# PTsolvers/JustRelax.jl

Measured on AMD Instinct MI355X. Metric: PT-iterations/s (3D Stokes SolVi3D, 512^3 fp64 block per GPU, block-iterations summed over GPUs), higher is better.
Workload: dtype f64; 1 GPU; SolVi3D 512^3 per GPU (configs[3]): eta inclusion 1e-3, G=1, K=Inf, dt=Inf, free-slip, pure shear; kernel_form=viscous_limit_no_body_forces, halo=none, arrays=library constructor, field_placement=1 (pool-dealt chunks, mapped once), operand_cache=0

## Files before the change

### justrelax.jl_amd/csrc/jrx_kernels.hpp

```cpp
#pragma once
#include "jrx_internal.hpp"

namespace {

__global__ __launch_bounds__(256) void k_scale3(double *__restrict__ U0, const double *__restrict__ V0, i64 n0,
                                                double *__restrict__ U1, const double *__restrict__ V1, i64 n1,
                                                double *__restrict__ U2, const double *__restrict__ V2, i64 n2, double dt)
{
    const i64 stride = (i64)gridDim.x * blockDim.x;
    for (i64 t = (i64)blockIdx.x * blockDim.x + threadIdx.x; t < n0 || t < n1 || t < n2; t += stride) {
        if (t < n0) U0[t] = V0[t] * dt;
        if (t < n1) U1[t] = V1[t] * dt;
        if (U2 && t < n2) U2[t] = V2[t] * dt;
    }
}

struct BcArr {
    double *p;
    int n[3];
};

__global__ __launch_bounds__(256) void k_bc3d(BcArr A0, BcArr A1, BcArr A2, int type, int dim, int lo_on, int hi_on)
{
    const BcArr arrs[3] = {A0, A1, A2};
// ... 19 lines not shown
                if (hi_on) p[base + (e - 1) * s[dim]] = 0.0;
            } else {
                if (lo_on) p[base] = -p[base + s[dim]];
                if (hi_on) p[base + (e - 1) * s[dim]] = -p[base + (e - 2) * s[dim]];
            }
        } else {
            if (normal) {
                if (lo_on) p[base] = p[base + (e - 1) * s[dim]];
            } else {
                if (lo_on) p[base] = p[base + (e - 2) * s[dim]];
                if (hi_on) p[base + (e - 1) * s[dim]] = p[base + s[dim]];
            }
        }
    }
}

struct CBcArr {
    const double *p;
    int n[3];
};
__global__ __launch_bounds__(256) void k_copy_shell3(BcArr D0, BcArr D1, BcArr D2, CBcArr S0, CBcArr S1, CBcArr S2)
{
    const BcArr D = blockIdx.z == 0 ? D0 : (blockIdx.z == 1 ? D1 : D2);
    const CBcArr S = blockIdx.z == 0 ? S0 : (blockIdx.z == 1 ? S1 : S2);
    const int dim = blockIdx.y >> 1, side = blockIdx.y & 1;
    const int d1 = dim == 0 ? 1 : 0, d2 = dim == 2 ? 1 : 2;
    const i64 u = (i64)blockIdx.x * blockDim.x + threadIdx.x;
    if (u >= (i64)D.n[d1] * D.n[d2]) return;
    const int a = (int)(u % D.n[d1]), b = (int)(u / D.n[d1]);
    const i64 s[3] = {1, D.n[0], (i64)D.n[0] * D.n[1]};
    const i64 idx = a * s[d1] + b * s[d2] + (side ? (i64)(D.n[dim] - 1) * s[dim] : 0);
    D.p[idx] = S.p[idx];
}

__global__ __launch_bounds__(256) void k_bc3d_faces(BcArr A0, BcArr A1, BcArr A2, int tlo0, int thi0, int tlo1, int thi1, int tlo2, int thi2)
{
    const BcArr arrs[3] = {A0, A1, A2};
    const int dim = blockIdx.z;
    const int tlo = dim == 0 ? tlo0 : (dim == 1 ? tlo1 : tlo2), thi = dim == 0 ? thi0 : (dim == 1 ? thi1 : thi2);
    if (!tlo && !thi) return;
    const int d1 = dim == 0 ? 1 : 0, d2 = dim == 2 ? 1 : 2;
    const int ta = blockIdx.x * blockDim.x + threadIdx.x;
    const int tb = blockIdx.y;
#pragma unroll
    for (int c = 0; c < 3; c++) {
        const BcArr &A = arrs[c];
        if (ta >= A.n[d1] || tb >= A.n[d2]) continue;
        const bool normal = (c == dim);
        const i64 s[3] = {1, A.n[0], (i64)A.n[0] * A.n[1]};
        const i64 base = ta * s[d1] + tb * s[d2];
        const int e = A.n[dim];
        double *p = A.p;
        if (normal) {
            if (tlo == 2) p[base] = 0.0;
            if (thi == 2) p[base + (e - 1) * s[dim]] = 0.0;
        } else {
            if (tlo == 1) p[base] = p[base + s[dim]];
            else if (tlo == 2) p[base] = -p[base + s[dim]];
            if (thi == 1) p[base + (e - 1) * s[dim]] = p[base + (e - 2) * s[dim]];
            else if (thi == 2) p[base + (e - 1) * s[dim]] = -p[base + (e - 2) * s[dim]];
        }
    }
}

__global__ __launch_bounds__(256) void k_maxloc(double *__restrict__ B, const double *__restrict__ A, int nx, int ny, int nz)
{
    const int t = blockIdx.x * blockDim.x + threadIdx.x;
    const int j = t / nx, i = t - j * nx, k = blockIdx.y;
    if (j >= ny) return;
    double x = -INFINITY;
    for (int kk = k - 1; kk <= k + 1; kk++) {
        const int kc = clampi(kk, 0, nz - 1);
        for (int jj = j - 1; jj <= j + 1; jj++) {
            const int jc = clampi(jj, 0, ny - 1);
            for (int ii = i - 1; ii <= i + 1; ii++) {
                const int ic = clampi(ii, 0, nx - 1);
                const double v = A[ic + (i64)nx * jc + (i64)nx * ny * kc];
                if (v > x) x = v;
            }
        }
    }
    B[i + (i64)nx * j + (i64)nx * ny * k] = x;
}

struct RedArr {
    const double *p;
    int n[3];
    int inner;
};

__global__ __launch_bounds__(256) void k_sumsq_partial(RedArr A0, RedArr A1, RedArr A2, RedArr A3, double *__restrict__ partials)
{
    const RedArr arrs[4] = {A0, A1, A2, A3};
    __shared__ double sm[4][4];
    const int lane = threadIdx.x & 63, wave = threadIdx.x >> 6;
    const i64 stride = (i64)gridDim.x * blockDim.x;
#pragma unroll
    for (int c = 0; c < 4; c++) {
        const RedArr &A = arrs[c];
        double s = 0.0;
        if (A.p) {
            const i64 n = (i64)A.n[0] * A.n[1] * A.n[2];
            for (i64 t = (i64)blockIdx.x * blockDim.x + threadIdx.x; t < n; t += stride) {
                bool take = true;
                if (A.inner) {
                    const int i = (int)(t % A.n[0]);
                    const i64 q = t / A.n[0];
                    const int j = (int)(q % A.n[1]);
                    const int k = (int)(q / A.n[1]);
                    take = i > 0 && i < A.n[0] - 1 && j > 0 && j < A.n[1] - 1 && (A.n[2] == 1 || (k > 0 && k < A.n[2] - 1));
                }
                if (take) {
                    const double v = A.p[t];
                    s += v * v;
                }
            }
        }
        s = wave_sum(s);
        if (lane == 0) sm[c][wave] = s;
    }
    __syncthreads();
    if (threadIdx.x < 4) {
        const int c = threadIdx.x;
        partials[(i64)blockIdx.x * 4 + c] = (sm[c][0] + sm[c][1]) + (sm[c][2] + sm[c][3]);
    }
}

__global__ __launch_bounds__(256) void k_sumsq_final(const double *__restrict__ partials, int nblocks, double *__restrict__ out)
{
    __shared__ double sm[4][4];
    const int lane = threadIdx.x & 63, wave = threadIdx.x >> 6;
#pragma unroll
    for (int c = 0; c < 4; c++) {
        double s = 0.0;
        for (int b = threadIdx.x; b < nblocks; b += blockDim.x) s += partials[(i64)b * 4 + c];
        s = wave_sum(s);
        if (lane == 0) sm[c][wave] = s;
    }
    __syncthreads();
    if (threadIdx.x < 4) {
        const int c = threadIdx.x;
        out[c] = (sm[c][0] + sm[c][1]) + (sm[c][2] + sm[c][3]);
    }
}

__global__ __launch_bounds__(256) void k_maxabs_partial(const double *__restrict__ A0, i64 n0, const double *__restrict__ A1, i64 n1,
                                                        const double *__restrict__ A2, i64 n2, double *__restrict__ partials)
{
    __shared__ double sm[3][4];
    const double *A[3] = {A0, A1, A2};
    const i64 n[3] = {n0, n1, n2};
    const int lane = threadIdx.x & 63, wave = threadIdx.x >> 6;
    const i64 stride = (i64)gridDim.x * blockDim.x;
#pragma unroll
    for (int c = 0; c < 3; c++) {
        double m = 0.0;
        if (A[c])
            for (i64 t = (i64)blockIdx.x * blockDim.x + threadIdx.x; t < n[c]; t += stride) {
                const double v = fabs(A[c][t]);
                m = (v > m || v != v) ? v : m;
            }
#pragma unroll
        for (int off = 32; off > 0; off >>= 1) {
            const double o = __shfl_down(m, off, 64);
            m = (o > m || o != o) ? o : m;
        }
// ... 69 lines not shown
```

### justrelax.jl_amd/csrc/stokes3d.hip

```cpp
#include <vector>
#include <cstdlib>
#include "jrx_internal.hpp"
#include "jrx_kernels.hpp"
#include "stokes3d_kernels.hpp"
#include "jrx_tuning.h"

namespace {

SweepArgs make_args(const jrx_stokes3d_fields *f, const double *etatau, const jrx_stokes3d_params *p)
{
    SweepArgs a;
    a.f = *f;
    a.o = Out10{f->P, f->txx, f->tyy, f->tzz, f->tyz, f->txz, f->txy, f->Vx, f->Vy, f->Vz};
    a.etatau = etatau;
    a._dx = p->_dx; a._dy = p->_dy; a._dz = p->_dz;
    a.dt = p->dt; a.r = p->r; a.theta_dtau = p->theta_dtau; a.eta_dtau = p->eta_dtau;
    a.L = make_lay((int)p->nx, (int)p->ny, (int)p->nz);
    a.i0 = a.j0 = a.k0 = 0;
    a.i1 = a.j1 = a.k1 = 0;
    return a;
}

jrx_status check_params(jrx_handle *h, const jrx_stokes3d_fields *f, const jrx_stokes3d_params *p)
{
    if (!h) return JRX_ERR_ARG;
    if (!f || !p) return jrx_fail(h, JRX_ERR_ARG, "null fields/params");
    JRX_TRY(jrx_check_device(h));
    if (p->nx < 3 || p->ny < 3 || p->nz < 3) return jrx_fail(h, JRX_ERR_ARG, "3D Stokes needs at least 3 cells per dimension");
    const double cells = (double)(p->nx + 2) * (double)(p->ny + 2) * (double)(p->nz + 2);
    if (cells >= 2147483647.0) return jrx_fail(h, JRX_ERR_UNSUPPORTED, "local block too large for 32-bit plane indices");
    const void *req[] = {f->P, f->P0, f->Q, f->Vx, f->Vy, f->Vz, f->txx, f->tyy, f->tzz, f->tyz, f->txz, f->txy,
                         f->toxx, f->toyy, f->tozz, f->toyz, f->toxz, f->toxy, f->eta, f->K, f->G, f->fx, f->fy, f->fz};
    for (const void *q : req)
        if (!q) return jrx_fail(h, JRX_ERR_ARG, "a required field pointer is NULL");
    return JRX_OK;
}

jrx_status check_diag(jrx_handle *h, const jrx_stokes3d_fields *f)
{
    const void *req[] = {f->divV, f->exx, f->eyy, f->ezz, f->eyz, f->exz, f->exy, f->RP, f->Rx, f->Ry, f->Rz, f->Ux, f->Uy, f->Uz};
    for (const void *q : req)
        if (!q) return jrx_fail(h, JRX_ERR_ARG, "a diagnostic field pointer (∇V, ε, R, U) is NULL");
    return JRX_OK;
}

jrx_status launch_stress_v1(jrx_handle *h, hipStream_t s, SweepArgs a, bool diag, int i0, int i1, int j0, int j1, int k0, int k1)
{
    if (i1 <= i0 || j1 <= j0 || k1 <= k0) return JRX_OK;
    a.i0 = i0; a.i1 = i1; a.j0 = j0; a.j1 = j1; a.k0 = k0; a.k1 = k1;
    const i64 plane = (i64)(i1 - i0) * (j1 - j0);
    dim3 grid((unsigned)((plane + 255) / 256), (unsigned)(k1 - k0));
    if (diag) hipLaunchKernelGGL(k_stress3d<true>, grid, dim3(256), 0, s, a);
    else hipLaunchKernelGGL(k_stress3d<false>, grid, dim3(256), 0, s, a);
    JRX_LAUNCH_CHECK(h);
    return JRX_OK;
}

jrx_status launch_velocity_v1(jrx_handle *h, hipStream_t s, SweepArgs a, bool diag, int i0, int i1, int j0, int j1, int k0, int k1)
{
    if (i1 <= i0 || j1 <= j0 || k1 <= k0) return JRX_OK;
    a.i0 = i0; a.i1 = i1; a.j0 = j0; a.j1 = j1; a.k0 = k0; a.k1 = k1;
    const i64 plane = (i64)(i1 - i0) * (j1 - j0);
    dim3 grid((unsigned)((plane + 255) / 256), (unsigned)(k1 - k0));
    if (diag) hipLaunchKernelGGL(k_velocity3d<true>, grid, dim3(256), 0, s, a);
    else hipLaunchKernelGGL(k_velocity3d<false>, grid, dim3(256), 0, s, a);
    JRX_LAUNCH_CHECK(h);
    return JRX_OK;
}

bool fits_u32(const Lay3 &L)
{
    const double m = (double)(L.nx + 2) * (double)(L.ny + 2) * (double)(L.nz + 2) * 8.0;
    return m < 4294967296.0;
}

template <class F>
__device__ __forceinline__ void scan_pairs(const double *__restrict__ p, i64 n, F f)
{
    if (n <= 0) return;
    const i64 stride = (i64)gridDim.x * blockDim.x, t0 = (i64)blockIdx.x * blockDim.x + threadIdx.x;
    const i64 head = (reinterpret_cast<uintptr_t>(p) & 15) ? 1 : 0;
    const double2 *__restrict__ q = reinterpret_cast<const double2 *>(p + head);
    const i64 m = n - head;
    for (i64 t = t0; t < (m >> 1); t += stride) { const double2 v = q[t]; f(v.x); f(v.y); }
    if (t0 == 0) { if (head) f(p[0]); if (m & 1) f(p[n - 1]); }
}
__global__ __launch_bounds__(256) void k_visc_operands_ok(const double *__restrict__ c0, const double *__restrict__ c1, const double *__restrict__ c2, const double *__restrict__ c3,
                                                          const double *__restrict__ c4, const double *__restrict__ eta, i64 nc, const double *__restrict__ K, const double *__restrict__ G,
                                                          const double *__restrict__ yz, i64 nyz, const double *__restrict__ xz, i64 nxz, const double *__restrict__ xy, i64 nxy, int *bad,
                                                          const unsigned long long *__restrict__ fx, const unsigned long long *__restrict__ fy, const unsigned long long *__restrict__ fz)
{
    bool b = false;
    unsigned long long bxy = 0, bz = 0;
    auto fin = [&](double v) { b |= !isfinite(v); };
    auto mod = [&](double v) { b |= (v != v) || v == 0.0; };
    scan_pairs(c0, nc, fin); scan_pairs(c1, nc, fin); scan_pairs(c2, nc, fin); scan_pairs(c3, nc, fin); scan_pairs(c4, nc, fin); scan_pairs(eta, nc, fin);
    scan_pairs(K, nc, mod); scan_pairs(G, nc, mod);
    scan_pairs(yz, nyz, fin); scan_pairs(xz, nxz, fin); scan_pairs(xy, nxy, fin);
    if (fx) {
        scan_pairs(reinterpret_cast<const double *>(fx), nc, [&](double v) { bxy |= (unsigned long long)__double_as_longlong(v); });
        scan_pairs(reinterpret_cast<const double *>(fy), nc, [&](double v) { bxy |= (unsigned long long)__double_as_longlong(v); });
        scan_pairs(reinterpret_cast<const double *>(fz), nc, [&](double v) { bz |= (unsigned long long)__double_as_longlong(v); });
    }
    if (__any(b) && (threadIdx.x & 63) == 0) atomicOr(bad, 1);
    if (fx) {
        const int m = (__any(bxy != 0) ? 2 : 0) | (__any(bz != 0) ? 4 : 0);
        if (m && (threadIdx.x & 63) == 0) atomicOr(bad, m);
    }
}

__global__ __launch_bounds__(256) void k_forces_zero(const unsigned long long *__restrict__ fx, const unsigned long long *__restrict__ fy, const unsigned long long *__restrict__ fz, i64 nc, int *bad)
{
    const i64 stride = (i64)gridDim.x * blockDim.x;
    unsigned long long bxy = 0, bz = 0;
    for (i64 t = (i64)blockIdx.x * blockDim.x + threadIdx.x; t < nc; t += stride) { bxy |= fx[t] | fy[t]; bz |= fz[t]; }
    const int m = (__any(bxy != 0) ? 2 : 0) | (__any(bz != 0) ? 4 : 0);
    if (m && (threadIdx.x & 63) == 0) atomicOr(bad, m);
}

static jrx_status visc_operands_local(jrx_handle *h, const jrx_stokes3d_fields *f, const jrx_stokes3d_params *p, bool forces);
jrx_status visc_operands_check(jrx_handle *h, const jrx_stokes3d_fields *f, const jrx_stokes3d_params *p, bool forces = true)
{
    JRX_TRY(visc_operands_local(h, f, p, forces));
    if (jrx_comm_active(h)) {
        double v[2] = {h->visc_ok ? 0.0 : 1.0, (double)(2 - h->nof)};
        JRX_TRY(jrx_allreduce_host(h, v, 2, 1));
        h->visc_ok = v[0] == 0.0;
        h->nof = 2 - (int)v[1];
    }
    return JRX_OK;
}
static jrx_status visc_operands_local(jrx_handle *h, const jrx_stokes3d_fields *f, const jrx_stokes3d_params *p, bool forces)
{
    h->visc_ok = false;
    h->nof = 0;
    forces = forces && h->zero_forces && f->fx && f->fy && f->fz;
    const void *key[14] = {f->P0, f->Q, f->toxx, f->toyy, f->tozz, f->toyz, f->toxz, f->toxy, f->eta, f->K, f->G, f->fx, f->fy, f->fz};
    const int kflags = (forces ? 1 : 0) | (h->viscous_limit ? 2 : 0) | (p->displacement_bcs ? 4 : 0) | (h->kernel_variant << 3);
    if (h->operand_cache && h->opv.valid && h->opv.dt == p->dt && h->opv.flags == kflags && h->opv.n[0] == p->nx && h->opv.n[1] == p->ny && h->opv.n[2] == p->nz &&
        memcmp(h->opv.ptr, key, sizeof(key)) == 0) {
        h->visc_ok = h->opv.visc_ok;
        h->nof = h->opv.nof;
        h->stat_operand_cache_hits++;
        return JRX_OK;
    }
    struct Remember {
        jrx_handle *h; const void *const *key; const jrx_stokes3d_params *p; int kflags; bool ok = false;
        ~Remember() {
            h->opv.valid = ok;
            if (!ok) return;
            memcpy(h->opv.ptr, key, sizeof(h->opv.ptr));
            h->opv.n[0] = p->nx; h->opv.n[1] = p->ny; h->opv.n[2] = p->nz; h->opv.dt = p->dt; h->opv.flags = kflags; h->opv.visc_ok = h->visc_ok; h->opv.nof = h->nof;
        }
    } remember{h, key, p, kflags};
    if ((!h->viscous_limit || p->dt != INFINITY) && forces && !p->displacement_bcs && (h->kernel_variant == 0 || h->kernel_variant == 3) && p->nx >= 48) {
        const i64 nc = (i64)p->nx * p->ny * p->nz;
        int *d_bad = reinterpret_cast<int *>(h->d_sums + 6), *h_bad = reinterpret_cast<int *>(h->h_sums + 6);
        hipStream_t s = h->stream;
        JRX_HIP(h, hipMemsetAsync(d_bad, 0, sizeof(double), s));
        hipLaunchKernelGGL(k_forces_zero, dim3(2048), dim3(256), 0, s, reinterpret_cast<const unsigned long long *>(f->fx), reinterpret_cast<const unsigned long long *>(f->fy),
                           reinterpret_cast<const unsigned long long *>(f->fz), nc, d_bad);
        JRX_LAUNCH_CHECK(h);
        JRX_HIP(h, hipMemcpyAsync(h_bad, d_bad, sizeof(double), hipMemcpyDeviceToHost, s));
        JRX_HIP(h, hipStreamSynchronize(s));
        if (!(*h_bad & 2)) h->nof = (*h_bad & 4) ? 1 : 2;
        remember.ok = true;
        return JRX_OK;
    }
    if (!h->viscous_limit || p->dt != INFINITY) { remember.ok = true; return JRX_OK; }
    const i64 nx = p->nx, ny = p->ny, nz = p->nz;
    int *d_bad = reinterpret_cast<int *>(h->d_sums + 6), *h_bad = reinterpret_cast<int *>(h->h_sums + 6);
    hipStream_t s = h->stream;
    JRX_HIP(h, hipMemsetAsync(d_bad, 0, sizeof(double), s));
    hipLaunchKernelGGL(k_visc_operands_ok, dim3(4096), dim3(256), 0, s, f->P0, f->Q, f->toxx, f->toyy, f->tozz, f->eta, nx * ny * nz, f->K, f->G, f->toyz, nx * (ny + 1) * (nz + 1),
                       f->toxz, (nx + 1) * ny * (nz + 1), f->toxy, (nx + 1) * (ny + 1) * nz, d_bad,
                       forces ? reinterpret_cast<const unsigned long long *>(f->fx) : nullptr, reinterpret_cast<const unsigned long long *>(f->fy), reinterpret_cast<const unsigned long long *>(f->fz));
    JRX_LAUNCH_CHECK(h);
    JRX_HIP(h, hipMemcpyAsync(h_bad, d_bad, sizeof(double), hipMemcpyDeviceToHost, s));
    JRX_HIP(h, hipStreamSynchronize(s));
    h->visc_ok = ((*h_bad & 1) == 0);
    if (h->visc_ok && forces && !(*h_bad & 2)) h->nof = (*h_bad & 4) ? 1 : 2;
    h->stat_visc_checks++;
    if (!h->visc_ok) h->stat_visc_fallbacks++;
    remember.ok = true;
    return JRX_OK;
}

template <int TX, int TY, int KZ>
jrx_status launch_stress_zb(jrx_handle *h, hipStream_t s, const SweepArgs &a, bool diag)
{
    const TileMap tm = make_tilemap(a.L.nx, a.L.ny, a.L.nz, TX, TY, KZ);
    if (diag) hipLaunchKernelGGL((k_stress3d_zb<true, TX, TY, KZ, 4, false, 8, true>), dim3(tm.ntiles), dim3(TX * TY), 0, s, a, tm);
    else if (h->viscous_limit && h->visc_ok && a.dt == INFINITY)
        hipLaunchKernelGGL((k_stress3d_zb<false, TX, TY, KZ, 4, false, 8, true, true>), dim3(tm.ntiles), dim3(TX * TY), 0, s, a, tm);
    else hipLaunchKernelGGL((k_stress3d_zb<false, TX, TY, KZ, 4, false, 8, true>), dim3(tm.ntiles), dim3(TX * TY), 0, s, a, tm);
    JRX_LAUNCH_CHECK(h);
    h->stat_sweeps3d++;
    return JRX_OK;
// ... 54 lines not shown

jrx_status launch_bcs(jrx_handle *h, hipStream_t s, double *Vx, double *Vy, double *Vz, int nx, int ny, int nz,
                      uint32_t fs, uint32_t ns, uint32_t pe)
{
    BcArr A[3] = {{Vx, {nx + 1, ny + 2, nz + 2}}, {Vy, {nx + 2, ny + 1, nz + 2}}, {Vz, {nx + 2, ny + 2, nz + 1}}};
    auto run = [&](int type, int dim, bool lo, bool hi) -> jrx_status {
        if (!lo && !hi) return JRX_OK;
        const int d1 = dim == 0 ? 1 : 0, d2 = dim == 2 ? 1 : 2;
        int na = 0, nb = 0;
        for (int c = 0; c < 3; c++) { na = A[c].n[d1] > na ? A[c].n[d1] : na; nb = A[c].n[d2] > nb ? A[c].n[d2] : nb; }
        hipLaunchKernelGGL(k_bc3d, dim3((na + 255) / 256, nb), dim3(256), 0, s, A[0], A[1], A[2], type, dim, (int)lo, (int)hi);
        JRX_LAUNCH_CHECK(h);
        return JRX_OK;
    };
    if (ns) {
        JRX_TRY(run(1, 0, ns & JRX_FACE_LEFT, ns & JRX_FACE_RIGHT));
        JRX_TRY(run(1, 1, ns & JRX_FACE_FRONT, ns & JRX_FACE_BACK));
        JRX_TRY(run(1, 2, ns & JRX_FACE_BOT, ns & JRX_FACE_TOP));
    }
    if (fs) {
        JRX_TRY(run(0, 1, fs & JRX_FACE_FRONT, fs & JRX_FACE_BACK));
        JRX_TRY(run(0, 2, fs & JRX_FACE_TOP, fs & JRX_FACE_BOT));
        JRX_TRY(run(0, 0, fs & JRX_FACE_LEFT, fs & JRX_FACE_RIGHT));
    }
    if (pe) {
        JRX_TRY(run(2, 0, pe & JRX_FACE_LEFT, pe & JRX_FACE_RIGHT));
        JRX_TRY(run(2, 1, pe & JRX_FACE_FRONT, pe & JRX_FACE_BACK));
        JRX_TRY(run(2, 2, pe & JRX_FACE_BOT, pe & JRX_FACE_TOP));
    }
    return JRX_OK;
}

static jrx_status launch_bcs_faces(jrx_handle *h, hipStream_t s, double *Vx, double *Vy, double *Vz, int nx, int ny, int nz, uint32_t fs, uint32_t ns)
{
    BcArr A[3] = {{Vx, {nx + 1, ny + 2, nz + 2}}, {Vy, {nx + 2, ny + 1, nz + 2}}, {Vz, {nx + 2, ny + 2, nz + 1}}};
    auto ty = [&](uint32_t fsbit, uint32_t nsbit) { return (ns & nsbit) ? 2 : ((fs & fsbit) ? 1 : 0); };
    const int t[6] = {ty(JRX_FACE_LEFT, JRX_FACE_LEFT), ty(JRX_FACE_RIGHT, JRX_FACE_RIGHT), ty(JRX_FACE_FRONT, JRX_FACE_FRONT),
                      ty(JRX_FACE_BACK, JRX_FACE_BACK), ty(JRX_FACE_TOP, JRX_FACE_BOT), ty(JRX_FACE_BOT, JRX_FACE_TOP)};
    if (!(t[0] | t[1] | t[2] | t[3] | t[4] | t[5])) return JRX_OK;
    const int na = (nx > ny ? nx : ny) + 2, nb = (ny > nz ? ny : nz) + 2;
    hipLaunchKernelGGL(k_bc3d_faces, dim3((na + 255) / 256, nb, 3), dim3(256), 0, s, A[0], A[1], A[2], t[0], t[1], t[2], t[3], t[4], t[5]);
    JRX_LAUNCH_CHECK(h);
    return JRX_OK;
}

static jrx_status launch_stress_boxes(jrx_handle *h, hipStream_t s, const SweepArgs &a, const int (*box)[6], int nbox, bool diag, const GhostRule *rule)
{
    StressBoxes B = {};
    int tot = 0;
    for (int q = 0; q < nbox; q++) {
        const int *b = box[q];
        if (b[1] <= b[0] || b[3] <= b[2] || b[5] <= b[4]) continue;
        const i64 plane = (i64)(b[1] - b[0]) * (b[3] - b[2]);
        for (int c = 0; c < 6; c++) B.box[B.n][c] = b[c];
        B.per_plane[B.n] = (int)((plane + 255) / 256);
        B.start[B.n] = tot;
        tot += B.per_plane[B.n] * (b[5] - b[4]);
        B.n++;
    }
    if (!B.n) return JRX_OK;
    B.start[B.n] = tot;
    const GhostRule none = {{0, 0, 0, 0, 0, 0}};
    const bool visc = !diag && h->viscous_limit && h->visc_ok && a.dt == INFINITY;
    if (rule && visc) hipLaunchKernelGGL((k_stress3d_boxes<false, true, true>), dim3((unsigned)tot), dim3(256), 0, s, a, B, *rule);
    else if (rule) hipLaunchKernelGGL((k_stress3d_boxes<false, true>), dim3((unsigned)tot), dim3(256), 0, s, a, B, *rule);
    else if (visc) hipLaunchKernelGGL((k_stress3d_boxes<false, false, true>), dim3((unsigned)tot), dim3(256), 0, s, a, B, none);
    else if (diag) hipLaunchKernelGGL(k_stress3d_boxes<true>, dim3((unsigned)tot), dim3(256), 0, s, a, B, none);
    else hipLaunchKernelGGL(k_stress3d_boxes<false>, dim3((unsigned)tot), dim3(256), 0, s, a, B, none);
    JRX_LAUNCH_CHECK(h);
    return JRX_OK;
}

jrx_status launch_sumsq(jrx_handle *h, hipStream_t s, const jrx_stokes3d_fields *f, const jrx_stokes3d_params *p)
{
    const int nx = (int)p->nx, ny = (int)p->ny, nz = (int)p->nz;
    RedArr A0 = {f->Rx, {nx - 1, ny, nz}, 1}, A1 = {f->Ry, {nx, ny - 1, nz}, 1}, A2 = {f->Rz, {nx, ny, nz - 1}, 1},
           A3 = {f->RP, {nx, ny, nz}, 0};
    const i64 n = (i64)nx * ny * nz;
    int nb = (int)((n + 256 * 8 - 1) / (256 * 8));
    nb = nb < 1 ? 1 : (nb > kMaxRedBlocks ? kMaxRedBlocks : nb);
    hipLaunchKernelGGL(k_sumsq_partial, dim3(nb), dim3(256), 0, s, A0, A1, A2, A3, h->d_partials);
    JRX_LAUNCH_CHECK(h);
    hipLaunchKernelGGL(k_sumsq_final, dim3(1), dim3(256), 0, s, h->d_partials, nb, h->d_sums);
    JRX_LAUNCH_CHECK(h);
    return JRX_OK;
}

}

jrx_status jrx3d_velocity_sweep(jrx_handle *h, hipStream_t s, const jrx_stokes3d_fields *f, const double *etatau, const jrx_stokes3d_params *p, bool diag, int nof)
{
    if (diag && (!f->Rx || !f->Ry || !f->Rz)) return jrx_fail(h, JRX_ERR_ARG, "residual arrays are NULL");
    return launch_velocity(h, s, make_args(f, etatau, p), diag, 0, (int)p->nx, 0, (int)p->ny, 0, (int)p->nz, nof);
}
jrx_status jrx3d_forces_zero(jrx_handle *h, hipStream_t s, const double *fx, const double *fy, const double *fz, int64_t nc, int *nof)
{
    *nof = 0;
    if (!h->zero_forces || !fx || !fy || !fz) return JRX_OK;
    int *d_bad = reinterpret_cast<int *>(h->d_sums + 6), *h_bad = reinterpret_cast<int *>(h->h_sums + 6);
    JRX_HIP(h, hipMemsetAsync(d_bad, 0, sizeof(double), s));
    hipLaunchKernelGGL(k_forces_zero, dim3(2048), dim3(256), 0, s, reinterpret_cast<const unsigned long long *>(fx), reinterpret_cast<const unsigned long long *>(fy),
                       reinterpret_cast<const unsigned long long *>(fz), (i64)nc, d_bad);
    JRX_LAUNCH_CHECK(h);
    JRX_HIP(h, hipMemcpyAsync(h_bad, d_bad, sizeof(double), hipMemcpyDeviceToHost, s));
    JRX_HIP(h, hipStreamSynchronize(s));
    if (!(*h_bad & 2)) *nof = (*h_bad & 4) ? 1 : 2;
    return JRX_OK;
}
jrx_status jrx3d_scaleU(jrx_handle *h, hipStream_t s, const jrx_stokes3d_fields *f, const jrx_stokes3d_params *p) { return launch_scaleU(h, s, f, p); }
jrx_status jrx3d_bcs(jrx_handle *h, hipStream_t s, double *Vx, double *Vy, double *Vz, int nx, int ny, int nz, uint32_t fs, uint32_t ns, uint32_t pe)
{
    return launch_bcs(h, s, Vx, Vy, Vz, nx, ny, nz, fs, ns, pe);
}
jrx_status jrx3d_sumsq(jrx_handle *h, hipStream_t s, const jrx_stokes3d_fields *f, const jrx_stokes3d_params *p) { return launch_sumsq(h, s, f, p); }
jrx_status jrx3d_bcs_faces(jrx_handle *h, hipStream_t s, double *Vx, double *Vy, double *Vz, int nx, int ny, int nz, uint32_t fs, uint32_t ns)
{
    return launch_bcs_faces(h, s, Vx, Vy, Vz, nx, ny, nz, fs, ns);
}

jrx_status jrx3d_velocity_hidden(jrx_handle *h, const jrx_stokes3d_fields *f, const double *etatau, const jrx_stokes3d_params *p, bool diag, int bc_kind)
{
    if (diag && (!f->Rx || !f->Ry || !f->Rz)) return jrx_fail(h, JRX_ERR_ARG, "residual arrays are NULL");
    const int nx = (int)p->nx, ny = (int)p->ny, nz = (int)p->nz;
    hipStream_t s = h->stream;
    const SweepArgs a = make_args(f, etatau, p);
    int bx = p->b_width[0] > 0 ? p->b_width[0] : 4, by = p->b_width[1] > 0 ? p->b_width[1] : 4,
        bz = p->b_width[2] > 0 ? p->b_width[2] : 4;
    if (h->b_width_opt[0] > 0) bx = h->b_width_opt[0];
    if (h->b_width_opt[1] > 0) by = h->b_width_opt[1];
    if (h->b_width_opt[2] > 0) bz = h->b_width_opt[2];
    const int xa = bx < nx / 2 ? bx : nx / 2, ya = by < ny / 2 ? by : ny / 2, za = bz < nz / 2 ? bz : nz / 2;
    hipStream_t hs = h->halo_stream;
    JRX_HIP(h, hipEventRecord(h->ev[0], s));
    JRX_HIP(h, hipStreamWaitEvent(hs, h->ev[0], 0));
    JRX_TRY(launch_velocity(h, hs, a, diag, 0, nx, 0, ny, 0, za));
    JRX_TRY(launch_velocity(h, hs, a, diag, 0, nx, 0, ny, nz - za, nz));
    JRX_TRY(launch_velocity(h, hs, a, diag, 0, nx, 0, ya, za, nz - za));
    JRX_TRY(launch_velocity(h, hs, a, diag, 0, nx, ny - ya, ny, za, nz - za));
    JRX_TRY(launch_velocity(h, hs, a, diag, 0, xa, ya, ny - ya, za, nz - za));
    JRX_TRY(launch_velocity(h, hs, a, diag, nx - xa, nx, ya, ny - ya, za, nz - za));
    JRX_TRY(launch_velocity(h, s, a, diag, xa, nx - xa, ya, ny - ya, za, nz - za));
    if (diag) {
        JRX_HIP(h, hipEventRecord(h->ev[1], s));
        JRX_HIP(h, hipStreamWaitEvent(hs, h->ev[1], 0));
        JRX_TRY(launch_scaleU(h, hs, f, p));
    }
    if (bc_kind == 0) JRX_TRY(launch_bcs(h, hs, f->Vx, f->Vy, f->Vz, nx, ny, nz, p->free_slip, p->no_slip, p->periodic));
    else if (bc_kind == 1) JRX_TRY(launch_bcs_faces(h, hs, f->Vx, f->Vy, f->Vz, nx, ny, nz, p->free_slip, p->no_slip));
    else if (bc_kind == 2) JRX_TRY(launch_bcs(h, hs, f->Ux, f->Uy, f->Uz, nx, ny, nz, p->free_slip, p->no_slip, p->periodic));
    double *arrs[3] = {f->Vx, f->Vy, f->Vz};
    const int64_t ext[3][3] = {{nx + 1, ny + 2, nz + 2}, {nx + 2, ny + 1, nz + 2}, {nx + 2, ny + 2, nz + 1}};
    const int64_t n[3] = {nx, ny, nz};
    JRX_TRY(jrx_halo_exchange(h, hs, 3, arrs, ext, n));
    JRX_HIP(h, hipEventRecord(h->ev[2], hs));
    JRX_HIP(h, hipStreamWaitEvent(s, h->ev[2], 0));
    return JRX_OK;
}

extern "C" {

jrx_status jrx_stokes3d_sweep_stress(jrx_handle *h, const jrx_stokes3d_fields *f, const jrx_stokes3d_params *p, int32_t flags)
{
    JRX_TRY(check_params(h, f, p));
    const bool diag = flags & JRX_OUT_DIAG;
    if (diag) JRX_TRY(check_diag(h, f));
    SweepArgs a = make_args(f, nullptr, p);
// ... 1 lines not shown
    else { h->visc_ok = false; h->nof = 0; }
    JRX_TRY(launch_stress(h, h->stream, a, diag, 0, (int)p->nx + 1, 0, (int)p->ny + 1, 0, (int)p->nz + 1));
    JRX_HIP(h, hipStreamSynchronize(h->stream));
    return JRX_OK;
}

jrx_status jrx_stokes3d_sweep_velocity(jrx_handle *h, const jrx_stokes3d_fields *f, const double *etatau,
                                       const jrx_stokes3d_params *p, int32_t flags)
{
    JRX_TRY(check_params(h, f, p));
    if (!etatau) return jrx_fail(h, JRX_ERR_ARG, "etatau is NULL");
    const bool diag = flags & JRX_OUT_DIAG;
    if (diag) JRX_TRY(check_diag(h, f));
    SweepArgs a = make_args(f, etatau, p);
    JRX_TRY(launch_velocity(h, h->stream, a, diag, 0, (int)p->nx, 0, (int)p->ny, 0, (int)p->nz));
    if (diag) JRX_TRY(launch_scaleU(h, h->stream, f, p));
    JRX_HIP(h, hipStreamSynchronize(h->stream));
    return JRX_OK;
}

jrx_status jrx_flow_bcs3d(jrx_handle *h, double *Vx, double *Vy, double *Vz, int64_t nx, int64_t ny, int64_t nz,
                          uint32_t free_slip, uint32_t no_slip, uint32_t periodic)
{
    if (!h) return JRX_ERR_ARG;
    if (!Vx || !Vy || !Vz) return jrx_fail(h, JRX_ERR_ARG, "null velocity pointer");
    JRX_TRY(launch_bcs(h, h->stream, Vx, Vy, Vz, (int)nx, (int)ny, (int)nz, free_slip, no_slip, periodic));
    JRX_HIP(h, hipStreamSynchronize(h->stream));
    return JRX_OK;
}

jrx_status jrx_stokes3d_residual_sumsq(jrx_handle *h, const jrx_stokes3d_fields *f, const jrx_stokes3d_params *p, double out[4])
{
    JRX_TRY(check_params(h, f, p));
    JRX_TRY(check_diag(h, f));
    JRX_TRY(launch_sumsq(h, h->stream, f, p));
    JRX_HIP(h, hipMemcpyAsync(h->h_sums, h->d_sums, 4 * sizeof(double), hipMemcpyDeviceToHost, h->stream));
    JRX_HIP(h, hipStreamSynchronize(h->stream));
    for (int c = 0; c < 4; c++) out[c] = h->h_sums[c];
    return JRX_OK;
}

jrx_status jrx_velocity2displacement(jrx_handle *h, double *const U[3], const double *const V[3], const int64_t n[3], double dt)
{
    if (!h) return JRX_ERR_ARG;
    if (!U || !V || !n || !U[0] || !U[1] || !V[0] || !V[1]) return jrx_fail(h, JRX_ERR_ARG, "velocity2displacement!: null argument");
    hipLaunchKernelGGL(k_scale3, dim3(2048), dim3(256), 0, h->stream, U[0], V[0], (i64)n[0], U[1], V[1], (i64)n[1], U[2], V[2], (i64)(U[2] ? n[2] : 0), dt);
    JRX_LAUNCH_CHECK(h);
    JRX_HIP(h, hipStreamSynchronize(h->stream));
    return JRX_OK;
}
jrx_status jrx_displacement2velocity(jrx_handle *h, double *const V[3], const double *const U[3], const int64_t n[3], double dt)
{
    return jrx_velocity2displacement(h, V, U, n, 1.0 / dt);
}

jrx_status jrx_compute_dt(jrx_handle *h, const double *const V[3], const int64_t n[3], const double di[3], int32_t ndim, double dt_diff, double *dt_out)
{
    if (!h) return JRX_ERR_ARG;
    if (!V || !n || !di || !dt_out || ndim < 2 || ndim > 3 || !V[0] || !V[1] || (ndim == 3 && !V[2])) return jrx_fail(h, JRX_ERR_ARG, "compute_dt: bad argument");
    i64 nmax = 0;
    for (int d = 0; d < ndim; d++) nmax = n[d] > nmax ? (i64)n[d] : nmax;
    int nb = (int)((nmax + 2047) / 2048);
    nb = nb < 1 ? 1 : (nb > kMaxRedBlocks ? kMaxRedBlocks : nb);
    hipStream_t s = h->stream;
    hipLaunchKernelGGL(k_maxabs_partial, dim3(nb), dim3(256), 0, s, V[0], (i64)n[0], V[1], (i64)n[1], ndim == 3 ? V[2] : (const double *)nullptr,
                       (i64)(ndim == 3 ? n[2] : 0), h->d_partials);
    hipLaunchKernelGGL(k_maxabs_final, dim3(1), dim3(256), 0, s, h->d_partials, nb, h->d_sums);
    JRX_LAUNCH_CHECK(h);
    JRX_HIP(h, hipMemcpyAsync(h->h_sums, h->d_sums, 4 * sizeof(double), hipMemcpyDeviceToHost, s));
    JRX_HIP(h, hipStreamSynchronize(s));
    double m[3] = {h->h_sums[0], h->h_sums[1], h->h_sums[2]};
    JRX_TRY(jrx_allreduce_host(h, m, ndim, 1));
    double dt_adv = INFINITY;
    for (int d = 0; d < ndim; d++) dt_adv = fmin(dt_adv, di[d] * (1.0 / m[d]));
    *dt_out = fmin(dt_diff, dt_adv * 0.9);
    return JRX_OK;
}

jrx_status jrx_compute_maxloc(jrx_handle *h, double *B, const double *A, int64_t nx, int64_t ny, int64_t nz)
{
    if (!h) return JRX_ERR_ARG;
    if (!A || !B || nx < 1 || ny < 1 || nz < 1) return jrx_fail(h, JRX_ERR_ARG, "bad compute_maxloc arguments");
    if (A == B) return jrx_fail(h, JRX_ERR_ARG, "compute_maxloc!: B must not alias A");
    const i64 plane = (i64)nx * ny;
    hipLaunchKernelGGL(k_maxloc, dim3((unsigned)((plane + 255) / 256), (unsigned)nz), dim3(256), 0, h->stream, B, A, (int)nx, (int)ny, (int)nz);
    JRX_LAUNCH_CHECK(h);
    JRX_HIP(h, hipStreamSynchronize(h->stream));
    return JRX_OK;
}

}

struct FusedShape { int tx, ty, kz; };
static void fused_tiles(const Lay3 &L, const FusedShape S, int nt[3])
{
    nt[0] = (L.nx + S.tx - 3) / (S.tx - 2); nt[1] = (L.ny + S.ty - 2) / (S.ty - 1); nt[2] = (L.nz + S.kz - 1) / S.kz;
}
static FusedShape fused_shape(const jrx_handle *h, const Lay3 &L, double dt)
{
    const bool narrow = h->fused_tile == 1 || (h->fused_tile == 2 && L.nx > 62 && L.nx <= 90);
    FusedShape S = narrow ? FusedShape{32, 8, 8} : FusedShape{64, 4, 8};
    int nt[3];
    {
        const int tkz = h->fused_kz == 8 || h->fused_kz == 12 ? h->fused_kz : (L.nz >= 384 ? 12 : 8);
        const FusedShape T{64, 8, tkz};
        fused_tiles(L, T, nt);
        const bool visc = h->viscous_limit && h->visc_ok && dt == INFINITY;
        if (h->fused_ylds && h->fused_tile == 4) return FusedShape{64, 16, 12};
        if (h->fused_ylds && (h->fused_tile == 3 || ((visc || L.nz >= 384) && h->fused_tile == 2 && !narrow && (long long)nt[0] * nt[1] * nt[2] >= 4096))) return T;
    }
    for (int kz = 8; kz >= 2; kz /= 2) {
        S.kz = kz;
        fused_tiles(L, S, nt);
        if ((long long)nt[0] * nt[1] * nt[2] >= 512) break;
    }
    return S;
}

struct Iter3D {
    jrx_handle *h;
    const jrx_stokes3d_params *p;
    const double *etatau;
    jrx_stokes3d_fields cur;
    Out10 setU, setS;
    bool pt_user = true, v_user = true;
    bool flip_A = false, flip_B = false;
    bool all_user() const { return pt_user && v_user; }
    bool stress_done = false;
    bool fusable = false;
    bool bcs_ordered[2] = {false, false};
    bool ghosts_stale = false;
};

static Out10 out_of(const jrx_stokes3d_fields &f) { return Out10{f.P, f.txx, f.tyy, f.tzz, f.tyz, f.txz, f.txy, f.Vx, f.Vy, f.Vz}; }
static void set_state(jrx_stokes3d_fields &f, const Out10 &o)
{
    f.P = o.P; f.txx = o.txx; f.tyy = o.tyy; f.tzz = o.tzz; f.tyz = o.tyz; f.txz = o.txz; f.txy = o.txy; f.Vx = o.Vx; f.Vy = o.Vy; f.Vz = o.Vz;
}
static Out10 mix_sets(const Out10 &pt, const Out10 &v) { return Out10{pt.P, pt.txx, pt.tyy, pt.tzz, pt.tyz, pt.txz, pt.txy, v.Vx, v.Vy, v.Vz}; }

static jrx_status ensure_scratch(jrx_handle *h, int nx, int ny, int nz)
{
    const size_t n[10] = {(size_t)nx * ny * nz, (size_t)nx * ny * nz, (size_t)nx * ny * nz, (size_t)nx * ny * nz,
                          (size_t)nx * (ny + 1) * (nz + 1), (size_t)(nx + 1) * ny * (nz + 1), (size_t)(nx + 1) * (ny + 1) * nz,
                          (size_t)(nx + 1) * (ny + 2) * (nz + 2), (size_t)(nx + 2) * (ny + 1) * (nz + 2), (size_t)(nx + 2) * (ny + 2) * (nz + 1)};
    if (h->scratch_dims[0] == nx && h->scratch_dims[1] == ny && h->scratch_dims[2] == nz && h->scratch[0] && h->scratch_stagger_used == h->scratch_stagger + 1000003 * (int)h->scratch_contiguous) return JRX_OK;
    for (int q = 0; q < 10; q++) {
        if (h->scratch_base[q]) JRX_TRY(jrx_dev_free(h, h->scratch_base[q]));
        h->scratch[q] = h->scratch_base[q] = nullptr;
    }
    h->scratch_dims[0] = h->scratch_dims[1] = h->scratch_dims[2] = 0;
    const size_t stg = (size_t)(h->scratch_stagger > 0 ? h->scratch_stagger : 0) & ~(size_t)255;
    for (int q = 0; q < 10; q++) {
        void *b = nullptr;
        const int keep = h->field_placement;
        if (h->scratch_contiguous) h->field_placement = 2;
        const jrx_status st = jrx_dev_alloc(h, n[q] * sizeof(double) + (size_t)q * stg, &b, 1);
        h->field_placement = keep;
        JRX_TRY(st);
        h->scratch_base[q] = (double *)b;
        h->scratch[q] = (double *)((char *)b + (size_t)q * stg);
    }
    h->scratch_stagger_used = h->scratch_stagger + 1000003 * (int)h->scratch_contiguous;
    h->scratch_dims[0] = nx; h->scratch_dims[1] = ny; h->scratch_dims[2] = nz;
    return JRX_OK;
}

static jrx_status iter_begin(Iter3D &I, jrx_handle *h, const jrx_stokes3d_fields *f, const double *etatau, const jrx_stokes3d_params *p)
{
// ... 428 lines not shown
        I.stress_done = true;
        if (was_fused) *was_fused = 1;
        if (tev) JRX_HIP(h, hipEventRecord(tev[2], s));
        return JRX_OK;
    }

    const jrx_stokes3d_fields *f = &I.cur;
    if (!jrx_comm_active(h)) {
        if (I.ghosts_stale && diag) {
            JRX_TRY(launch_bcs(h, s, f->Vx, f->Vy, f->Vz, nx, ny, nz, p->free_slip, p->no_slip, p->periodic));
            I.bcs_ordered[I.v_user ? 0 : 1] = true;
        }
        I.ghosts_stale = false;
        if (I.flip_B && !p->displacement_bcs) {
            const Out10 other = mix_sets(I.pt_user ? I.setU : I.setS, I.v_user ? I.setS : I.setU);
            a.o = other;
            JRX_TRY(launch_velocity(h, s, a, diag, 0, nx, 0, ny, 0, nz, h->nof));
            set_state(I.cur, other);
            I.v_user = !I.v_user;
        } else
            JRX_TRY(launch_velocity(h, s, a, diag, 0, nx, 0, ny, 0, nz, h->nof));
        I.flip_B = false;
        if (tev) JRX_HIP(h, hipEventRecord(tev[2], s));
        if (diag) JRX_TRY(launch_scaleU(h, s, f, p));
        if (p->displacement_bcs) {
            if (diag) JRX_TRY(launch_bcs(h, s, f->Ux, f->Uy, f->Uz, nx, ny, nz, p->free_slip, p->no_slip, p->periodic));
            return JRX_OK;
        }
        bool &ordered = I.bcs_ordered[I.v_user ? 0 : 1];
        if (!diag && ordered && p->periodic == 0) JRX_TRY(launch_bcs_faces(h, s, f->Vx, f->Vy, f->Vz, nx, ny, nz, p->free_slip, p->no_slip));
        else {
            JRX_TRY(launch_bcs(h, s, f->Vx, f->Vy, f->Vz, nx, ny, nz, p->free_slip, p->no_slip, p->periodic));
            ordered = true;
        }
        return JRX_OK;
    }
    if (I.ghosts_stale) {
        uint32_t fs_keep, ns_keep;
        physical_faces(h, &fs_keep, &ns_keep);
        JRX_TRY(launch_bcs(h, s, f->Vx, f->Vy, f->Vz, nx, ny, nz, p->free_slip & fs_keep, p->no_slip & ns_keep, 0));
        I.ghosts_stale = false;
    }
    return jrx3d_velocity_hidden(h, f, I.etatau, p, diag, p->displacement_bcs ? (diag ? 2 : 3) : 0);
}

static jrx_status iter_end(Iter3D &I)
{
    jrx_handle *h = I.h;
    if (I.stress_done) return jrx_fail(h, JRX_ERR_ARG, "internal: iteration pipeline ended with a pending fused stress sweep");
    if (I.all_user()) return JRX_OK;
    const jrx_stokes3d_params *p = I.p;
    const i64 nc = (i64)p->nx * p->ny * p->nz, nyz = (i64)p->nx * (p->ny + 1) * (p->nz + 1), nxz = (i64)(p->nx + 1) * p->ny * (p->nz + 1),
              nxy = (i64)(p->nx + 1) * (p->ny + 1) * p->nz, n0 = (i64)(p->nx + 1) * (p->ny + 2) * (p->nz + 2),
              n1 = (i64)(p->nx + 2) * (p->ny + 1) * (p->nz + 2), n2 = (i64)(p->nx + 2) * (p->ny + 2) * (p->nz + 1);
    const Out10 &S = I.setS, &U = I.setU;
    const i64 zp = I.pt_user ? 0 : 1, zv = I.v_user ? 0 : 1;
    if (zp) {
        hipLaunchKernelGGL(k_copy6, dim3(2048), dim3(256), 0, h->stream, U.P, (const double *)S.P, nc, U.txx, (const double *)S.txx, nc, U.tyy,
                           (const double *)S.tyy, nc, U.tzz, (const double *)S.tzz, nc, U.tyz, (const double *)S.tyz, nyz, U.txz, (const double *)S.txz, nxz);
        JRX_LAUNCH_CHECK(h);
    }
    hipLaunchKernelGGL(k_copy6, dim3(2048), dim3(256), 0, h->stream, U.txy, (const double *)S.txy, nxy * zp, U.Vx, (const double *)S.Vx, n0 * zv, U.Vy,
                       (const double *)S.Vy, n1 * zv, U.Vz, (const double *)S.Vz, n2 * zv, (double *)nullptr, (const double *)nullptr, (i64)0, (double *)nullptr,
                       (const double *)nullptr, (i64)0);
    JRX_LAUNCH_CHECK(h);
    set_state(I.cur, U);
    I.pt_user = I.v_user = true;
    return JRX_OK;
}

extern "C" {

jrx_status jrx_stokes3d_solve(jrx_handle *h, const jrx_stokes3d_fields *f, const jrx_stokes3d_params *p, jrx_solve_result *res)
{
    JRX_TRY(check_params(h, f, p));
    JRX_TRY(check_diag(h, f));
    if (!res) return jrx_fail(h, JRX_ERR_ARG, "null result");
    if (p->nout < 1) return jrx_fail(h, JRX_ERR_ARG, "nout must be >= 1");
    const int nx = (int)p->nx, ny = (int)p->ny, nz = (int)p->nz;
    const size_t n = (size_t)nx * ny * nz;
    hipStream_t s = h->stream;

    JRX_TRY(jrx_ensure_etatau(h, n));
    hipLaunchKernelGGL(k_maxloc, dim3((unsigned)(((i64)nx * ny + 255) / 256), (unsigned)nz), dim3(256), 0, s, h->etatau, f->eta, nx, ny, nz);
    JRX_LAUNCH_CHECK(h);
    if (jrx_comm_active(h)) {
        double *arrs[1] = {h->etatau};
        const int64_t ext[1][3] = {{nx, ny, nz}};
        const int64_t nn[3] = {nx, ny, nz};
        JRX_TRY(jrx_halo_exchange(h, s, 1, arrs, ext, nn));
    }

    if (p->displacement_bcs) {
        hipLaunchKernelGGL(k_scale3, dim3(2048), dim3(256), 0, s, f->Vx, (const double *)f->Ux, (i64)(nx + 1) * (ny + 2) * (nz + 2), f->Vy,
                           (const double *)f->Uy, (i64)(nx + 2) * (ny + 1) * (nz + 2), f->Vz, (const double *)f->Uz, (i64)(nx + 2) * (ny + 2) * (nz + 1),
                           1.0 / p->dt);
        JRX_LAUNCH_CHECK(h);
    }
    PtLog log(res);
    int64_t iter = 0;
    res->iter = 0; res->nchecks = 0;
    const int rank = jrx_comm_rank(h);
    hipEvent_t t0 = h->ev[6], t1 = h->ev[7];
    Iter3D I;
    JRX_TRY(iter_begin(I, h, f, h->etatau, p));
    JRX_HIP(h, hipEventRecord(t0, s));
    auto keep_going = [&](int64_t it) { return it < 2 || ((log.rel() > p->eps_rel && log.err() > p->eps_abs) && it <= p->iterMax); };
    auto is_check = [&](int64_t it1) { return (it1 % p->nout == 0) && it1 > 1; };
    constexpr int GIT = 16;
    GraphExecs gexec;
    bool graphs = h->loop_graphs && !I.fusable && !jrx_comm_active(h) && !p->displacement_bcs && p->periodic == 0 && (double)n <= kGraphCells3D;
    while (keep_going(iter)) {
        if (graphs && iter >= 2 && I.bcs_ordered[0] && I.all_user() && !I.stress_done) {
            int64_t nxt = ((iter / p->nout) + 1) * p->nout;
            if (nxt > p->iterMax + 1) nxt = p->iterMax + 1;
            int64_t run = nxt - 1 - iter;
            if (run >= GIT) {
                if (!gexec[0]) {
                    JRX_TRY(jrx_capture_graph(s, &gexec[0], [&]() -> jrx_status {
                        for (int q = 0; q < GIT; q++) JRX_TRY(iter_step(I, false, false, nullptr, nullptr));
                        return JRX_OK;
                    }));
                    if (!gexec[0]) graphs = false;
                }
                if (gexec[0]) {
                    while (run >= GIT) {
                        JRX_HIP(h, hipGraphLaunch(gexec[0], s));
                        iter += GIT; run -= GIT;
                        h->stat_graph_replays++;
                    }
                    continue;
                }
            }
        }
        const int64_t it1 = iter + 1;
        const bool check = is_check(it1);
        const bool diag = check || !keep_going(it1);
        const bool fuse_next = !diag && keep_going(it1) && !(is_check(it1 + 1) || !keep_going(it1 + 1));
        JRX_TRY(iter_step(I, diag, fuse_next, nullptr, nullptr));
        iter = it1;
        if (check) {
            JRX_TRY(launch_sumsq(h, s, &I.cur, p));
            double ss[4];
            JRX_TRY(jrx_read_sums(h, s, ss, true));
            const double nRx = sqrt(ss[0]) / (double)((p->nxg - 2) * (p->nyg - 1) * (p->nzg - 1));
            const double nRy = sqrt(ss[1]) / (double)((p->nxg - 1) * (p->nyg - 2) * (p->nzg - 1));
            const double nRz = sqrt(ss[2]) / (double)((p->nxg - 1) * (p->nyg - 1) * (p->nzg - 2));
            const double nDV = sqrt(ss[3]) / (double)(p->nxg * p->nyg * p->nzg);
            const double err = log.record(iter, nRx, nRy, nRz, nDV);
            if (rank == 0 && ((p->verbose && log.rel() > p->eps_rel && err > p->eps_abs) || iter == p->iterMax)) log.print3d(iter, nRx, nRy, nRz, nDV);
            if (std::isnan(err)) {
                (void)iter_end(I);
                return log.fail_nan(h, iter, jrx_drain_ms(s, t0, t1));
            }
        }
    }
    JRX_HIP(h, hipEventRecord(t1, s));
    JRX_TRY(iter_end(I));
    JRX_TRY((jrx3d_copy_old_stresses<2048>(h, s, f, nx, ny, nz)));
    JRX_HIP(h, hipStreamSynchronize(s));
    float ms = 0.f;
    JRX_HIP(h, hipEventElapsedTime(&ms, t0, t1));
    log.finish(iter, ms);
    return JRX_OK;
}

jrx_status jrx_stokes3d_iterate_timed(jrx_handle *h, const jrx_stokes3d_fields *f, const double *etatau,
                                      const jrx_stokes3d_params *p, int64_t iters, double times_ms[6])
{
    JRX_TRY(check_params(h, f, p));
    if (!etatau) return jrx_fail(h, JRX_ERR_ARG, "etatau is NULL");
    if (iters < 1) return jrx_fail(h, JRX_ERR_ARG, "iters must be >= 1");
    if (!times_ms) return jrx_fail(h, JRX_ERR_ARG, "times_ms is NULL");
    hipStream_t s = h->stream;
    const int64_t stride = iters > 64 ? (((iters + 63) / 64) | 1) : 1;
    const int nsamp = (int)((iters + stride - 1) / stride);
    const bool chain = h->chain_profile && jrx_comm_active(h);
    std::vector<hipEvent_t> evs((size_t)nsamp * (chain ? 8 : 4));
    std::vector<int> fused((size_t)nsamp, 0), cmode((size_t)nsamp, 0);
    std::vector<double> ncell((size_t)nsamp, 0.0);
    struct EvGuard { std::vector<hipEvent_t> &v; ~EvGuard() { for (auto &e : v) if (e) (void)hipEventDestroy(e); } } guard{evs};
    for (auto &e : evs) e = nullptr;
    for (auto &e : evs) JRX_HIP(h, hipEventCreate(&e));
    Iter3D I;
    JRX_TRY(iter_begin(I, h, f, etatau, p));
    JRX_HIP(h, hipStreamSynchronize(s));
    JRX_HIP(h, hipEventRecord(h->ev[6], s));
    const bool odd = I.fusable && iters >= 2 && ((iters - 1) % 2 == 1);
    const bool flips = odd && h->end_flips && !jrx_comm_active(h) && p->periodic == 0 && !p->displacement_bcs;
    const bool first_unfused = odd && !flips;
    for (int64_t it = 0; it < iters; it++) {
        const bool samp = it % stride == 0;
        const bool fuse_next = it + 1 < iters && !(first_unfused && it == 0);
        if (flips && it == 0) I.flip_A = true;
        if (flips && it == iters - 1) I.flip_B = true;
        const size_t q = (size_t)(it / stride);
        JRX_TRY(iter_step(I, false, fuse_next, samp ? &evs[q * 4] : nullptr, samp ? &fused[q] : nullptr, samp ? &ncell[q] : nullptr,
                          samp && chain ? &evs[(size_t)nsamp * 4 + q * 4] : nullptr, samp && chain ? &cmode[q] : nullptr));
    }
    JRX_HIP(h, hipEventRecord(h->ev[7], s));
    JRX_TRY(iter_end(I));
    JRX_HIP(h, hipStreamSynchronize(s));
    float ms = 0.f;
    JRX_HIP(h, hipEventElapsedTime(&ms, h->ev[6], h->ev[7]));
    times_ms[0] = ms; times_ms[1] = times_ms[2] = times_ms[3] = times_ms[4] = times_ms[5] = 0.0;
    double sa = 0.0, sb = 0.0, sf = 0.0, sk = 0.0, sc = 0.0;
    int na = 0, nb = 0, nf = 0;
    const bool comm = jrx_comm_active(h);
    for (int q = 0; q < nsamp; q++) {
        if (comm && !fused[q]) continue;
        float m1 = 0.f, m2 = 0.f;
        JRX_HIP(h, hipEventElapsedTime(&m1, evs[(size_t)q * 4], evs[(size_t)q * 4 + 1]));
        JRX_HIP(h, hipEventElapsedTime(&m2, evs[(size_t)q * 4 + 1], evs[(size_t)q * 4 + 2]));
        if (fused[q]) {
            float m3 = 0.f;
            JRX_HIP(h, hipEventElapsedTime(&m3, evs[(size_t)q * 4 + 1], evs[(size_t)q * 4 + 3]));
            sf += m2; sk += m3; sc += ncell[q]; nf++;
        }
        else { sb += m2; nb++; }
        if (m1 > 1e-3f) { sa += m1; na++; }
    }
    if (chain) {
        double acc[8] = {0, 0, 0, 0, 0, 0, 0, 0};
        int nc = 0;
        auto el = [&](hipEvent_t a, hipEvent_t b) { float m = 0.f; (void)hipEventElapsedTime(&m, a, b); return (double)m * 1e3; };
        for (int q = 0; q < nsamp; q++) {
            if (!fused[q] || !cmode[q]) continue;
            hipEvent_t *t = &evs[(size_t)q * 4], *c = &evs[(size_t)nsamp * 4 + (size_t)q * 4];
            const double step = el(t[1], t[2]), kern = el(t[1], t[3]);
            if (cmode[q] == 2) {
                const double post = fmin(el(t[3], c[3]), el(c[2], c[3]));
                acc[0] += kern; acc[1] += el(t[1], c[0]); acc[2] += el(c[0], c[1]); acc[3] += el(c[1], c[2]); acc[4] += post; acc[5] += el(c[3], t[2]);
            } else {
                acc[0] += kern; acc[2] += el(t[3], c[1]); acc[3] += el(c[1], c[2]); acc[5] += el(c[2], t[2]);
            }
            acc[6] += step; acc[7] += step - kern;
            nc++;
        }
        for (int q = 0; q < 8; q++) h->chain_us[q] = nc ? acc[q] / nc : 0.0;
        h->chain_n = nc;
        (void)hipGetLastError();
    }
    if (na) times_ms[1] = sa / na;
    if (nb) times_ms[2] = sb / nb;
    if (nf) { times_ms[3] = sf / nf; times_ms[4] = sk / nf; times_ms[5] = sc / nf; }
    return JRX_OK;
}

}
```

Before: 210.8 it/s.

## Add z-marching maxloc kernel with shuffle reuse, unroll operand scans, resample profiling

Replaces the 27-point clamped maxloc stencil with a kernel that marches along z, reusing per-plane 3x3 maxima from a rolling window and using wavefront shuffles for x neighbours. Operand-check scans are unrolled four-wide with vectorized double2 loads, and the force-zero check now reuses that scan. The profiling loop takes fewer event samples and always samples the last iteration, tracking which samples own the A phase. The maxloc and checks run during setup rather than in the iteration loop, so their effect on per-iteration throughput is likely small. The reduced event sampling may slightly cut per-iteration overhead.

Result: no change. 210.2 it/s (-0.3%).

```diff
diff --git a/justrelax.jl_amd/csrc/jrx_kernels.hpp b/justrelax.jl_amd/csrc/jrx_kernels.hpp
--- a/justrelax.jl_amd/csrc/jrx_kernels.hpp
+++ b/justrelax.jl_amd/csrc/jrx_kernels.hpp
@@ -125,6 +125,50 @@
     }
     B[i + (i64)nx * j + (i64)nx * ny * k] = x;
 }
+__global__ __launch_bounds__(256) void k_maxloc_zm(double *__restrict__ B, const double *__restrict__ A, int nx, int ny, int nz, int kz)
+{
+    const i64 plane = (i64)nx * ny;
+    const i64 t = (i64)blockIdx.x * blockDim.x + threadIdx.x;
+    const bool valid = t < plane;
+    const i64 tc = valid ? t : plane - 1;
+    const int j = (int)(tc / nx), i = (int)(tc - (i64)j * nx);
+    const int lane = (int)(threadIdx.x & 63);
+    const bool xl = i > 0, xr = i < nx - 1;
+    const i64 rm = (i64)nx * clampi(j - 1, 0, ny - 1) + i, rc = (i64)nx * j + i, rp = (i64)nx * clampi(j + 1, 0, ny - 1) + i;
+    auto row_max = [&](const double *__restrict__ r) {
+        const double c = r[0];
+        double lo = __shfl_up(c, 1, 64), hi = __shfl_down(c, 1, 64);
+        if (lane == 0 && xl) lo = r[-1];
+        if (lane == 63 && xr) hi = r[1];
+        if (!xl) lo = c;
+        if (!xr) hi = c;
+        double x = -INFINITY;
+        if (lo > x) x = lo;
+        if (c > x) x = c;
+        if (hi > x) x = hi;
+        return x;
+    };
+    auto plane_max = [&](int kk) {
+        const double *__restrict__ Ak = A + plane * clampi(kk, 0, nz - 1);
+        const double m0 = row_max(Ak + rm), m1 = row_max(Ak + rc), m2 = row_max(Ak + rp);
+        double x = -INFINITY;
+        if (m0 > x) x = m0;
+        if (m1 > x) x = m1;
+        if (m2 > x) x = m2;
+        return x;
+    };
+    const int k0 = (int)blockIdx.y * kz, k1 = k0 + kz < nz ? k0 + kz : nz;
+    double mp = plane_max(k0 - 1), mc = plane_max(k0);
+    for (int k = k0; k < k1; k++) {
+        const double mn = plane_max(k + 1);
+        double x = -INFINITY;
+        if (mp > x) x = mp;
+        if (mc > x) x = mc;
+        if (mn > x) x = mn;
+        if (valid) B[t + plane * k] = x;
+        mp = mc; mc = mn;
+    }
+}
 
 struct RedArr {
     const double *p;
diff --git a/justrelax.jl_amd/csrc/stokes3d.hip b/justrelax.jl_amd/csrc/stokes3d.hip
--- a/justrelax.jl_amd/csrc/stokes3d.hip
+++ b/justrelax.jl_amd/csrc/stokes3d.hip
@@ -81,8 +81,13 @@
     const i64 stride = (i64)gridDim.x * blockDim.x, t0 = (i64)blockIdx.x * blockDim.x + threadIdx.x;
     const i64 head = (reinterpret_cast<uintptr_t>(p) & 15) ? 1 : 0;
     const double2 *__restrict__ q = reinterpret_cast<const double2 *>(p + head);
-    const i64 m = n - head;
-    for (i64 t = t0; t < (m >> 1); t += stride) { const double2 v = q[t]; f(v.x); f(v.y); }
+    const i64 m = n - head, m2 = m >> 1;
+    i64 t = t0;
+    for (; t + 3 * stride < m2; t += 4 * stride) {
+        const double2 v0 = q[t], v1 = q[t + stride], v2 = q[t + 2 * stride], v3 = q[t + 3 * stride];
+        f(v0.x); f(v0.y); f(v1.x); f(v1.y); f(v2.x); f(v2.y); f(v3.x); f(v3.y);
+    }
+    for (; t < m2; t += stride) { const double2 v = q[t]; f(v.x); f(v.y); }
     if (t0 == 0) { if (head) f(p[0]); if (m & 1) f(p[n - 1]); }
 }
 __global__ __launch_bounds__(256) void k_visc_operands_ok(const double *__restrict__ c0, const double *__restrict__ c1, const double *__restrict__ c2, const double *__restrict__ c3,
@@ -111,9 +116,10 @@
 
 __global__ __launch_bounds__(256) void k_forces_zero(const unsigned long long *__restrict__ fx, const unsigned long long *__restrict__ fy, const unsigned long long *__restrict__ fz, i64 nc, int *bad)
 {
-    const i64 stride = (i64)gridDim.x * blockDim.x;
     unsigned long long bxy = 0, bz = 0;
-    for (i64 t = (i64)blockIdx.x * blockDim.x + threadIdx.x; t < nc; t += stride) { bxy |= fx[t] | fy[t]; bz |= fz[t]; }
+    scan_pairs(reinterpret_cast<const double *>(fx), nc, [&](double v) { bxy |= (unsigned long long)__double_as_longlong(v); });
+    scan_pairs(reinterpret_cast<const double *>(fy), nc, [&](double v) { bxy |= (unsigned long long)__double_as_longlong(v); });
+    scan_pairs(reinterpret_cast<const double *>(fz), nc, [&](double v) { bz |= (unsigned long long)__double_as_longlong(v); });
     const int m = (__any(bxy != 0) ? 2 : 0) | (__any(bz != 0) ? 4 : 0);
     if (m && (threadIdx.x & 63) == 0) atomicOr(bad, m);
 }
@@ -334,6 +340,19 @@
     hipLaunchKernelGGL(k_sumsq_partial, dim3(nb), dim3(256), 0, s, A0, A1, A2, A3, h->d_partials);
     JRX_LAUNCH_CHECK(h);
     hipLaunchKernelGGL(k_sumsq_final, dim3(1), dim3(256), 0, s, h->d_partials, nb, h->d_sums);
+    JRX_LAUNCH_CHECK(h);
+    return JRX_OK;
+}
+
+jrx_status launch_maxloc(jrx_handle *h, hipStream_t s, double *B, const double *A, int nx, int ny, int nz)
+{
+    const unsigned gx = (unsigned)(((i64)nx * ny + 255) / 256);
+    if (nz == 1) hipLaunchKernelGGL(k_maxloc, dim3(gx, 1), dim3(256), 0, s, B, A, nx, ny, nz);
+    else {
+        int kz = 8;
+        while (kz > 1 && (i64)gx * ((nz + kz - 1) / kz) < 1024) kz /= 2;
+        hipLaunchKernelGGL(k_maxloc_zm, dim3(gx, (unsigned)((nz + kz - 1) / kz)), dim3(256), 0, s, B, A, nx, ny, nz, kz);
+    }
     JRX_LAUNCH_CHECK(h);
     return JRX_OK;
 }
@@ -501,9 +520,7 @@
     if (!h) return JRX_ERR_ARG;
     if (!A || !B || nx < 1 || ny < 1 || nz < 1) return jrx_fail(h, JRX_ERR_ARG, "bad compute_maxloc arguments");
     if (A == B) return jrx_fail(h, JRX_ERR_ARG, "compute_maxloc!: B must not alias A");
-    const i64 plane = (i64)nx * ny;
-    hipLaunchKernelGGL(k_maxloc, dim3((unsigned)((plane + 255) / 256), (unsigned)nz), dim3(256), 0, h->stream, B, A, (int)nx, (int)ny, (int)nz);
-    JRX_LAUNCH_CHECK(h);
+    JRX_TRY(launch_maxloc(h, h->stream, B, A, (int)nx, (int)ny, (int)nz));
     JRX_HIP(h, hipStreamSynchronize(h->stream));
     return JRX_OK;
 }
@@ -1098,8 +1115,7 @@
     hipStream_t s = h->stream;
 
     JRX_TRY(jrx_ensure_etatau(h, n));
-    hipLaunchKernelGGL(k_maxloc, dim3((unsigned)(((i64)nx * ny + 255) / 256), (unsigned)nz), dim3(256), 0, s, h->etatau, f->eta, nx, ny, nz);
-    JRX_LAUNCH_CHECK(h);
+    JRX_TRY(launch_maxloc(h, s, h->etatau, f->eta, nx, ny, nz));
     if (jrx_comm_active(h)) {
         double *arrs[1] = {h->etatau};
         const int64_t ext[1][3] = {{nx, ny, nz}};
@@ -1189,11 +1205,12 @@
     if (iters < 1) return jrx_fail(h, JRX_ERR_ARG, "iters must be >= 1");
     if (!times_ms) return jrx_fail(h, JRX_ERR_ARG, "times_ms is NULL");
     hipStream_t s = h->stream;
-    const int64_t stride = iters > 64 ? (((iters + 63) / 64) | 1) : 1;
-    const int nsamp = (int)((iters + stride - 1) / stride);
+    const int64_t stride = iters > 8 ? (((iters + 6) / 7) | 1) : 1;
+    const int nstr = (int)((iters + stride - 1) / stride);
+    const int nsamp = nstr + ((iters - 1) % stride != 0 ? 1 : 0);
     const bool chain = h->chain_profile && jrx_comm_active(h);
     std::vector<hipEvent_t> evs((size_t)nsamp * (chain ? 8 : 4));
-    std::vector<int> fused((size_t)nsamp, 0), cmode((size_t)nsamp, 0);
+    std::vector<int> fused((size_t)nsamp, 0), cmode((size_t)nsamp, 0), own_a((size_t)nsamp, 0);
     std::vector<double> ncell((size_t)nsamp, 0.0);
     struct EvGuard { std::vector<hipEvent_t> &v; ~EvGuard() { for (auto &e : v) if (e) (void)hipEventDestroy(e); } } guard{evs};
     for (auto &e : evs) e = nullptr;
@@ -1206,11 +1223,12 @@
     const bool flips = odd && h->end_flips && !jrx_comm_active(h) && p->periodic == 0 && !p->displacement_bcs;
     const bool first_unfused = odd && !flips;
     for (int64_t it = 0; it < iters; it++) {
-        const bool samp = it % stride == 0;
+        const bool samp = it % stride == 0 || it == iters - 1;
         const bool fuse_next = it + 1 < iters && !(first_unfused && it == 0);
         if (flips && it == 0) I.flip_A = true;
         if (flips && it == iters - 1) I.flip_B = true;
-        const size_t q = (size_t)(it / stride);
+        const size_t q = it % stride == 0 ? (size_t)(it / stride) : (size_t)nsamp - 1;
+        if (samp) own_a[q] = !I.stress_done;
         JRX_TRY(iter_step(I, false, fuse_next, samp ? &evs[q * 4] : nullptr, samp ? &fused[q] : nullptr, samp ? &ncell[q] : nullptr,
                           samp && chain ? &evs[(size_t)nsamp * 4 + q * 4] : nullptr, samp && chain ? &cmode[q] : nullptr));
     }
@@ -1234,7 +1252,7 @@
             sf += m2; sk += m3; sc += ncell[q]; nf++;
         }
         else { sb += m2; nb++; }
-        if (m1 > 1e-3f) { sa += m1; na++; }
+        if (own_a[q]) { sa += m1; na++; }
     }
     if (chain) {
         double acc[8] = {0, 0, 0, 0, 0, 0, 0, 0};
```
